# jmabuin/metacache-mpi

Hardware: AMD Instinct MI355X
Metric: query reads/sec (whole node) (higher is better)
Workload: dtype u32; 1 GPU; BASELINE configs[1]: 500 synthetic genomes (50 species x 10 strains, 2.0% divergence, 1.96 Gbp) in HBM, 1048576 x 150 bp single-end reads per step per GPU, k=16 s=16 w=128/113; reads_total=1632632832, db_keys=94389458, db_locations=277440620, db_hbm_bytes=34394191464, db_scaling=fixed, emulate_ranks=2, max_cand=2, P_x_M=4, distinct_batches=321, db_targets=500, parallelism=1 GPU, db_build_parts=1, remove_overpopulated_features=False

## Files before the change

### metacache-mpi_amd/csrc/mcq_device.hpp

```cpp
#pragma once
#include <cstddef>
#include <hip/hip_runtime.h>
#include <stdint.h>

typedef uint32_t u32;
typedef uint64_t u64;

#define MCQ_EMPTY 0xFFFFFFFFu
#ifndef MCQ_BLOCK_LONG_FIRST
#define MCQ_BLOCK_LONG_FIRST 16384u
#endif
#define MCQ_Q_UNPROBED 0x80000000u
#define MCQ_MAX_FOLD 64
#define MCQ_BIGLIST_MAX 1024u

namespace mcq {

struct DbDev {
    const uint4* slots;
    u32 slot_mask;
    u32 bsh;
    const void* locs;
    u32 wb;
    u32 compact;
// ... 51 lines not shown
        }
        t = lo; tb = o;
    }
    __device__ __forceinline__ u32 tbeg(u32 k) const { u32 t, tb; locate(k, t, tb); return tb; }
    __device__ __forceinline__ u32 tgt(u32 k) const { u32 t, tb; locate(k, t, tb); return t; }
};
template <class KeyT, bool GW> struct LocOf { typedef LocShift<KeyT> type; };
template <> struct LocOf<u32, true> { typedef LocGW type; };
template <class KeyT, bool GW>
__device__ __forceinline__ typename LocOf<KeyT, GW>::type loc_format(const DbDev& db, const GwDev& g) {
    if constexpr (GW) { LocGW f; f.off = g.off; f.blk = reinterpret_cast<const uint2*>(g.blk); f.shift = g.shift; return f; }
    else { LocShift<KeyT> f; f.wb = db.wb; return f; }
}
template <class KeyT>
__device__ __forceinline__ KeyT range_low(KeyT k, KeyT tb, u32 numWindows) {
    return (k - tb >= (KeyT)numWindows) ? k - (KeyT)(numWindows - 1) : tb;
}

struct BatchDev {
    const char* bases;
    const u64* seq_off;
    u64 n_seq;
    u64 nq;
    u32 paired;
    u32 ranges;
    u32 packed;
    u32 amb_off;
    u32 last_word;
    u32 amb_last;
};
__device__ __forceinline__ void seq_bounds(const u64* seq_off, u32 ranges, u64 a, u64& beg, u64& end) {
    if (ranges) { beg = seq_off[2 * a]; end = seq_off[2 * a + 1]; }
    else { beg = seq_off[a]; end = seq_off[a + 1]; }
}

struct OptDev {
    u32 max_cand;
    u32 P;
    u32 seg;
    u32 big;
    u32 quirk_seq_drop;
    u32 hooks;
    u64 insert_size_max;
    u32 n_fold;
    u32 n_levels;
    unsigned char level_end[8];
    unsigned char fold_snd[MCQ_MAX_FOLD];
    unsigned char fold_rcv[MCQ_MAX_FOLD];
    u64 tc_limit;
    u32 lin;
    u32 keep;
};
enum : u32 {
    MCQ_HOOK_BLOCK_ONLY   = 1u,
    MCQ_HOOK_RAW_SORT     = 2u,
    MCQ_HOOK_NO_WAVE16    = 4u,
    MCQ_HOOK_ROUTE        = MCQ_HOOK_BLOCK_ONLY | MCQ_HOOK_RAW_SORT | MCQ_HOOK_NO_WAVE16,
    MCQ_HOOK_ONLY_LAUNCH  = 8u,
    MCQ_HOOK_NO_TWO_CLASS = 16u,
    MCQ_HOOK_STOP_SHIFT   = 8u,
};
__device__ __host__ __forceinline__ bool two_class_lists(const OptDev& opt) {
    return (opt.lin ? opt.P <= 8u : opt.P * opt.max_cand <= 16u) && !(opt.hooks & MCQ_HOOK_NO_TWO_CLASS);
}

struct OutDev {
// ... 163 lines not shown
    static constexpr u32 W = MCQ_GEOM_DEFAULT_WINLEN, S = MCQ_GEOM_DEFAULT_STRIDE;
    __device__ __forceinline__ explicit GeomDefault(const DbDev&) {}
    __device__ __forceinline__ static constexpr u32 k() { return MCQ_GEOM_DEFAULT_K; }
    __device__ __forceinline__ static constexpr u32 s() { return MCQ_GEOM_DEFAULT_S; }
    __device__ __forceinline__ static constexpr u32 winlen() { return W; }
    __device__ __forceinline__ static constexpr u32 winstride() { return S; }
    __device__ __forceinline__ static constexpr u32 tgt_winstride() { return S; }
    __device__ __forceinline__ static u32 num_windows(u32 n) {
        if (n <= W) return 1;
        const u32 nfull = (n - W) / S + 1;
        return nfull + ((nfull * S < n) ? 1u : 0u);
    }
    __device__ __forceinline__ static void window_of(u32 n, u32 j, u32& beg, u32& len) {
        if (n <= W) { beg = 0; len = n; return; }
        const u32 nfull = (n - W) / S + 1;
        beg = j * S;
        len = (j < nfull) ? W : (n - beg);
    }
    __device__ __forceinline__ static u32 range_width(u64 qlen, u64 insert_size_max) {
        const u64 m = qlen > insert_size_max ? qlen : insert_size_max;
        if (m < (1ull << 31)) return 2 + (u32)m / S;
        return (u32)(2 + m / S);
    }
};
inline bool geom_is_default(const DbDev& d) {
    return d.k == MCQ_GEOM_DEFAULT_K && d.s == MCQ_GEOM_DEFAULT_S && d.winlen == MCQ_GEOM_DEFAULT_WINLEN &&
           d.winstride == MCQ_GEOM_DEFAULT_STRIDE && d.tgt_winstride == MCQ_GEOM_DEFAULT_STRIDE;
}
struct BatchRt {
    const BatchDev& b;
    __device__ __forceinline__ explicit BatchRt(const BatchDev& x) : b(x) {}
    __device__ __forceinline__ bool paired() const { return b.paired != 0; }
    __device__ __forceinline__ bool packed() const { return b.packed != 0; }
};
template <bool PAIRED, bool PACKED>
struct BatchForm {
    __device__ __forceinline__ explicit BatchForm(const BatchDev&) {}
    __device__ __forceinline__ static constexpr bool paired() { return PAIRED; }
    __device__ __forceinline__ static constexpr bool packed() { return PACKED; }
};

__device__ __forceinline__ u32 lane_rank(u64 mask) {
    return __builtin_amdgcn_mbcnt_hi((u32)(mask >> 32), __builtin_amdgcn_mbcnt_lo((u32)mask, 0u));
}

__device__ __forceinline__ void wave_sync() {
    __builtin_amdgcn_fence(__ATOMIC_RELEASE, "wavefront");
    __builtin_amdgcn_wave_barrier();
    __builtin_amdgcn_fence(__ATOMIC_ACQUIRE, "wavefront");
}

template <int CTRL>
__device__ __forceinline__ u32 dpp_mov(u32 v) {
    return (u32)__builtin_amdgcn_mov_dpp((int)v, CTRL, 0xF, 0xF, false);
}

__device__ __forceinline__ u32 wave_min_u32(u32 v) {
    u32 t;
    t = dpp_mov<0xB1>(v);  v = t < v ? t : v;
    t = dpp_mov<0x4E>(v);  v = t < v ? t : v;
    t = dpp_mov<0x141>(v); v = t < v ? t : v;
    t = dpp_mov<0x140>(v); v = t < v ? t : v;
    u32 a = __builtin_amdgcn_readlane(v, 0), b = __builtin_amdgcn_readlane(v, 16);
    u32 c = __builtin_amdgcn_readlane(v, 32), d = __builtin_amdgcn_readlane(v, 48);
    a = a < b ? a : b; c = c < d ? c : d;
    return a < c ? a : c;
}

__device__ __forceinline__ u32 bcast(u32 v, u32 src_lane) {
    return __builtin_amdgcn_readlane(v, src_lane);
}

// ... 295 lines not shown
    if (F(b).packed()) wave_words_of_packed(b, at, lane, w, am);
    else { u32 c0, c1; window_chars(b.bases + at, n, lane, c0, c1); wave_words_of_chars(c0, c1, lane, w, am); }
    return wave_sketch_words(w, am, n, k, s, lane, tmp, dst);
}

#ifndef MCQ_SKETCH_EXPECT_FUSED
#define MCQ_SKETCH_EXPECT_FUSED 25
#endif
struct __attribute__((packed)) PackedU32 { u32 v; };
__device__ __forceinline__ void encode_chars4(u32 c, u32& code8, u32& amb4) {
    const u32 z = (c & 0xDFDFDFDFu) ^ 0x41414141u;
    const u32 r = (z >> 1) & 0x03030303u;
    const u32 t = r & ~(r << 1) & 0x02020202u;
    const u32 bad = (z & 0xF9F9F9F9u) ^ ((t >> 1) | (t << 3));
    const u32 f = ((((bad & 0x7F7F7F7Fu) + 0x7F7F7F7Fu) | bad) >> 7) & 0x01010101u;
    const u32 x = r ^ ((r >> 1) & 0x01010101u);
    const u32 px = (x << 2) | (x >> 8);
    code8 = ((px << 4) | (px >> 16)) & 0xFFu;
    const u32 pf = (f << 1) | (f >> 8);
    amb4 = ((pf << 2) | (pf >> 16)) & 0xFu;
}
template <bool WIDE>
__device__ __forceinline__ u32 sketch_sorted_prefix(const u32* tmp, u32 cnt, u32 cap, u32 lane, u32* dst) {
    u32 v = lane < cnt ? tmp[lane] : MCQ_EMPTY;
    v = WIDE ? wave_sort64_1(v) : wave_sort_blocks32_1(v);
    asm("s_nop 1" : "+v"(v));
    const u32 prev = (u32)__builtin_amdgcn_update_dpp(0, (int)v, 0x138, 0xF, 0xF, false);
    const bool keep = (v != MCQ_EMPTY) && (lane == 0 || v != prev);
    const u64 km = __ballot(keep);
    const u32 rank = lane_rank(km);
    if (keep && rank < cap) dst[rank] = v;
    return (u32)__builtin_popcountll(km);
}
template <u32 E = MCQ_SKETCH_EXPECT_FUSED, bool REMAT = false>
__device__ __forceinline__ u32 wave_sketch_two_windows(const char* __restrict__ seq, u32 n, u32 lane, u32* tmp, u32* dst, u32& path) {
    if constexpr (REMAT) asm volatile("" : "+v"(lane));
    constexpr u32 K = MCQ_GEOM_DEFAULT_K, S = MCQ_GEOM_DEFAULT_S, W = MCQ_GEOM_DEFAULT_WINLEN, ST = MCQ_GEOM_DEFAULT_STRIDE;
    static_assert(K == 16 && S == 16 && W == 128 && ST == W - K + 1, "the two windows' k-mers partition; a k-mer is one 32-bit word");
    const u32 p4 = 4 * lane;
    const u32 la = p4 < n - 4 ? p4 : n - 4;
    u32 c = reinterpret_cast<const PackedU32*>(seq + la)->v >> (8 * ((p4 - la) & 3u));
    if (p4 >= n) c = 0;
    u32 code8, amb4;
    encode_chars4(c, code8, amb4);
    u32 w = code8 << (24 - 8 * (lane & 3));
    w |= xor_lane<1>(w, lane); w |= xor_lane<2>(w, lane);
    u32 am = amb4 << (28 - 4 * (lane & 7));
    am |= xor_lane<1>(am, lane); am |= xor_lane<2>(am, lane); am |= xor_lane<4>(am, lane);
    const u32 sh = (lane & 15) * 2, ash = lane & 31;
    const u32 wsrc = (lane & 0x30u), asrc = (lane & 0x20u);
    u32 h[3];
#pragma unroll
    for (int i = 0; i < 3; ++i) {
        const u32 pos = lane + 64 * i;
        const u32 w0 = (u32)__builtin_amdgcn_ds_bpermute((int)(wsrc + 64 * i), (int)w);
        const u32 w1 = (u32)__builtin_amdgcn_ds_bpermute((int)(wsrc + 64 * i + 16), (int)w);
        const u32 kmer = (u32)((((u64)w0 << 32) | w1) >> (32 - sh));
        const u32 m0 = (u32)__builtin_amdgcn_ds_bpermute((int)(asrc + 64 * i), (int)am);
        const u32 m1 = (u32)__builtin_amdgcn_ds_bpermute((int)(asrc + 64 * i + 32), (int)am);
        const u32 amb32 = (u32)((((u64)m0 << 32) | m1) >> (32 - ash));
        const bool ok = (i == 0 || pos + K <= n) && (amb32 >> (32 - K)) == 0;
        h[i] = ok ? tmh(canonical(kmer, K)) : MCQ_EMPTY;
    }
    const bool b1 = lane >= ST - 64;
    const u32 ha0 = h[0], ha1 = b1 ? MCQ_EMPTY : h[1], hb = b1 ? h[1] : h[2];
    const u32 cA = (u32)__builtin_popcountll(__ballot(ha0 != MCQ_EMPTY)) + (u32)__builtin_popcountll(__ballot(ha1 != MCQ_EMPTY));
    const bool all_in = cA <= 32;
    const u32 thr = all_in ? MCQ_EMPTY : (u32)fminf(__builtin_amdgcn_rcpf((float)cA) * (4294967296.0f * E), 4294967040.0f);
    const bool s0 = ha0 < thr, s1 = ha1 < thr, sb = hb != MCQ_EMPTY;
    const u64 m0 = __ballot(s0), m1 = __ballot(s1), mb = __ballot(sb);
    const u32 n0 = (u32)__builtin_popcountll(m0), cntA = n0 + (u32)__builtin_popcountll(m1), cntB = (u32)__builtin_popcountll(mb);
    const u32 capB = n - W;
    const u32 slB = capB < S ? capB : S;
    path = 0;
    if (cntA <= 32) {
        if (s0) tmp[lane_rank(m0)] = ha0;
        if (s1) tmp[n0 + lane_rank(m1)] = ha1;
        if (sb) tmp[32 + lane_rank(mb)] = hb;
        wave_sync();
        const bool hi = lane >= 32;
        u32 v = lane < (hi ? 32 + cntB : cntA) ? tmp[lane] : MCQ_EMPTY;
        v = wave_sort_blocks32_1(v);
        asm("s_nop 1" : "+v"(v));
        const u32 prev = (u32)__builtin_amdgcn_update_dpp(0, (int)v, 0x138, 0xF, 0xF, false);
        const bool keep = (v != MCQ_EMPTY) && ((lane & 31) == 0 || v != prev);
        const u64 km = __ballot(keep);
        const u32 DA = (u32)__builtin_popcount((u32)km), DB = (u32)__builtin_popcount((u32)(km >> 32));
        if (all_in || DA >= S) {
            const u32 mA = DA < S ? DA : S, mB = DB < slB ? DB : slB;
            const u32 rank = lane_rank(km) - (hi ? DA : 0u);
            if (keep && rank < (hi ? mB : mA)) dst[rank + (hi ? mA : 0u)] = v;
            wave_sync();
            return mA + mB;
        }
        wave_sync();
    }
    u32 mA = 0;
    bool exact = cntA > 64 || cntA <= 32;
    if (!exact) {
        path = 1;
        if (s0) tmp[lane_rank(m0)] = ha0;
        if (s1) tmp[n0 + lane_rank(m1)] = ha1;
        wave_sync();
        const u32 DA = sketch_sorted_prefix<true>(tmp, cntA, S, lane, dst);
        if (DA < S) exact = true; else mA = S;
        wave_sync();
    }
    if (exact) {
        path = 2;
        u32 a0 = ha0, a1 = ha1;
        for (mA = 0; mA < S; ++mA) {
            const u32 lo = a0 < a1 ? a0 : a1;
            const u32 mn = wave_min_u32(lo);
            if (mn == MCQ_EMPTY) break;
            if (lane == 0) dst[mA] = mn;
            if (a0 == mn) a0 = MCQ_EMPTY;
            if (a1 == mn) a1 = MCQ_EMPTY;
        }
// ... 1151 lines not shown
```

### metacache-mpi_amd/csrc/mcq_engine.hip

```cpp
#include "mcq_internal.hpp"

static thread_local std::string g_err;
extern "C" const char* mcq_last_error(void) { return g_err.c_str(); }
int mcq::set_error(int code, const char* msg) { g_err = msg; return code; }
extern "C" const char* mcq_version(void) { return "mcq 0.1 (gfx950)"; }

template <class Kernel>
static u32 resident_blocks(Kernel kernel, int block_size, int device) {
    int per_cu = 0;
    hipDeviceProp_t prop;
    if (hipOccupancyMaxActiveBlocksPerMultiprocessor(&per_cu, kernel, block_size, 0) != hipSuccess || per_cu < 1) per_cu = 4;
    if (hipGetDeviceProperties(&prop, device) != hipSuccess || prop.multiProcessorCount < 1) prop.multiProcessorCount = 256;
    if (const char* e = getenv("MCQ_WAVE_BLOCKS_PER_CU")) per_cu = std::max(1, atoi(e));
    return std::min<u32>((u32)per_cu * (u32)prop.multiProcessorCount, 8192u);
}
static u32 grid_for(u32 cap, u64 want) { return (u32)std::min<u64>(want ? want : 1, cap ? cap : 1); }

#define MCQ_LCAP_WAVE16 1024
__device__ __forceinline__ u32 pow2ceil(u32 x) { return x <= 1 ? 1u : 1u << (32 - __builtin_clz(x - 1)); }

template <class KeyT> __device__ __forceinline__ KeyT key_pad() { return ~(KeyT)0; }
template <class KeyT, class LF> __device__ __forceinline__ u64 key_expand(KeyT k, const LF& lf) {
    u32 t; KeyT tb;
    lf.locate(k, t, tb);
// ... 119 lines not shown
        if (D <= 64) return topk_lin_write<u32, 9, LF::lookup>(db, opt, out, sk, H, D, lf, q, lane, t1);
        return topk_lin_write<u32, 9>(db, opt, out, sk, H, D, lf, q, lane);
    }
    if (D > 64) {
        u32 nheads = 0;
        for (u32 base = 0; base < D; base += 64) {
            const u32 j = base + lane;
            const u32 hv = (j < D) ? H[j] : 0;
            const u64 hm = __ballot(hv != 0);
            if (hv != 0) H[nheads + lane_rank(hm)] = hv;
            nheads += (u32)__builtin_popcountll(hm);
        }
        wave_sync();
        return topk_all_lds<9, 4>(db, opt, out, sk, H, nheads, numWindows, lf, q, lane, H + 256);
    }
    return topk_fold_write_lds<9, LF::lookup>(db, opt, out, sk, H, D, numWindows, lf, q, lane, H + 256, t1);
}
#ifdef MCQ_PHASE_CLOCK
__shared__ u64 g_wph[4][12];
#define WCLK(i) do { asm volatile("s_waitcnt vmcnt(0) lgkmcnt(0)" ::: "memory"); if ((threadIdx.x & 63) == 0) { const u64 t_ = __builtin_amdgcn_s_memtime(); \
    u64* p_ = g_wph[threadIdx.x >> 6]; p_[i] += t_ - p_[11]; p_[11] = t_; } } while (0)
#else
#define WCLK(i) do { } while (0)
#endif
__device__ __forceinline__ u32 dedup_slot(u32 key) { return (key * 0x9E3779B1u) >> 23; }
__device__ __forceinline__ u32* dedup_sk(u32* hits) { return hits + 256; }
__device__ __forceinline__ u32* dedup_wp(u32* hits) { return hits; }
__device__ __forceinline__ u32 dedup_count(const u32* tabkey, const u32* tabcnt, u32 k) {
    u32 slot = dedup_slot(k);
    while (tabkey[slot] != k) slot = (slot + 1) & 511u;
    return (tabcnt[slot >> 1] >> (16 * (slot & 1))) & 0xFFFFu;
}

template <int E>
__device__ __forceinline__ u32 dedup_insert(const u32 (&r)[E], u32* buf, u32* hits, u32 T, u32 lane) {
    u32* tabkey = buf; u32* tabcnt = hits; u32* list = hits + 256;
    reinterpret_cast<uint4*>(tabkey)[lane] = make_uint4(MCQ_EMPTY, MCQ_EMPTY, MCQ_EMPTY, MCQ_EMPTY);
    reinterpret_cast<uint4*>(tabkey)[64 + lane] = make_uint4(MCQ_EMPTY, MCQ_EMPTY, MCQ_EMPTY, MCQ_EMPTY);
    u32 zero;
    asm volatile("v_mov_b32 %0, 0" : "=v"(zero));
    reinterpret_cast<uint4*>(tabcnt)[lane] = make_uint4(zero, zero, zero, zero);
    wave_sync();
    u32 D = 0;
#pragma unroll
    for (int e = 0; e < E; ++e) {
        if (e > 0 && (u32)(e * 64) >= T) break;
        const u32 key = r[e];
        bool created = false;
        if ((u32)(e * 64) + lane < T) {
            u32 slot = dedup_slot(key);
            while (true) {
                const u32 old = atomicCAS(&tabkey[slot], MCQ_EMPTY, key);
                created = old == MCQ_EMPTY;
                if (created || old == key) { atomicAdd(&tabcnt[slot >> 1], 1u << (16 * (slot & 1))); break; }
                slot = (slot + 1) & 511u;
            }
        }
        const u64 cm = __ballot(created);
        const u32 rank = D + lane_rank(cm);
        if (created && rank < MCQ_DEDUP_MAX_D) list[rank] = key;
        D += (u32)__builtin_popcountll(cm);
        if (D > MCQ_DEDUP_MAX_D) break;
    }
    wave_sync();
    return D;
}
template <class LF>
__device__ __forceinline__ u32 dedup_finish(u32 D, u32* buf, u32* hits, u32 lane, const LF& lf, u32& k1, u32& incl1, u32& t1, u32& tb1) {
    u32* tabkey = buf; u32* tabcnt = hits; u32* list = hits + 256; u32* SK = dedup_sk(hits); u32* WP = dedup_wp(hits);
    k1 = MCQ_EMPTY; incl1 = 0; t1 = 0; tb1 = 0;
    if (D > MCQ_DEDUP_MAX_D) return ~0u;
// ... 3 lines not shown
        if constexpr (LF::lookup) lf.locate(lane < D ? k : list[0], t1, tb1);
        const u32 c = lane < D ? dedup_count(tabkey, tabcnt, k) : 0u;
        const u32 incl = wave_incl_scan_dpp(c);
        wave_sync();
        SK[lane] = k; WP[lane] = incl;
        k1 = k; incl1 = incl;
    } else if (D <= 128) {
        u32 k[2];
        k[0] = list[lane]; k[1] = (64 + lane < D) ? list[64 + lane] : MCQ_EMPTY;
        wave_regsort<u32, 2>(k, lane);
        const u32 c0 = dedup_count(tabkey, tabcnt, k[0]);
        const u32 c1 = (64 + lane < D) ? dedup_count(tabkey, tabcnt, k[1]) : 0u;
        const u32 i0 = wave_incl_scan_dpp(c0);
        const u32 i1 = wave_incl_scan_dpp(c1) + bcast(i0, 63);
        wave_sync();
        SK[lane] = k[0]; SK[64 + lane] = k[1]; WP[lane] = i0; WP[64 + lane] = i1;
    } else {
        u32 k[4], c[4];
#pragma unroll
        for (int e = 0; e < 4; ++e) k[e] = ((u32)(64 * e) + lane < D) ? list[64 * e + lane] : MCQ_EMPTY;
        wave_regsort<u32, 4>(k, lane);
#pragma unroll
        for (int e = 0; e < 4; ++e) c[e] = ((u32)(64 * e) + lane < D) ? dedup_count(tabkey, tabcnt, k[e]) : 0u;
        u32 carry = 0;
#pragma unroll
        for (int e = 0; e < 4; ++e) { c[e] = wave_incl_scan_dpp(c[e]) + carry; carry = bcast(c[e], 63); }
        wave_sync();
#pragma unroll
        for (int e = 0; e < 4; ++e) { SK[64 * e + lane] = k[e]; WP[64 * e + lane] = c[e]; }
    }
    wave_sync();
    return D;
}
template <int E>
__device__ __forceinline__ u32 gather_dedup_insert(const DbDev& db, u32* buf, u32* hits, u32 T, u32 pos, u32 len, u64 off, u32 lane, int stop) {
    u32 r[E];
    gather_regs<u32, E>(db, r, T, pos, len, off, lane, hits);
    if (stop == 3) {
        u32 x = 0;
#pragma unroll
        for (int e = 0; e < E; ++e) x ^= r[e];
        buf[lane] = x;
        return ~1u;
    }
    return dedup_insert<E>(r, buf, hits, T, lane);
}
template <int E>
__device__ __forceinline__ u32 gather2_dedup_insert(const DbDev& db, u32* buf, u32* hits, u32 T, u32 pos0, u32 len0, u64 off0,
                                                    u32 pos1, u32 len1, u64 off1, bool two, u32 lane) {
    u32 r[E];
    gather_regs2<E>(db, r, T, pos0, len0, off0, pos1, len1, off1, two, lane, hits);
    return dedup_insert<E>(r, buf, hits, T, lane);
}
template <int E>
__device__ __forceinline__ u32 load_dedup_insert(const u32* __restrict__ src, u32* buf, u32* hits, u32 T, u32 lane) {
    u32 r[E];
#pragma unroll
    for (int e = 0; e < E; ++e) { const u32 t = e * 64 + lane; r[e] = t < T ? src[t] : MCQ_EMPTY; }
    return dedup_insert<E>(r, buf, hits, T, lane);
}

template <int E, class LF>
__device__ __forceinline__ bool heavy_sweep(u32 nH, u32 numWindows, const LF& lf, u32 lane, u32* buf, u32* hits, u32& D, u32*& SK, u32*& H, bool& nine) {
    constexpr int JB = 10;
    D = 0; SK = dedup_sk(hits); H = buf; nine = true;
    if (nH) {
        u32 rh[E];
#pragma unroll
        for (int e = 0; e < E; ++e) { const u32 t = e * 64 + lane; rh[e] = t < nH ? hits[t] : MCQ_EMPTY; }
        wave_sync();
        u32 k1 = MCQ_EMPTY, incl1 = 0, t1 = 0, tb1 = 0;
        const u32 Dd = dedup_insert<E>(rh, buf, hits, nH, lane);
        WCLK(4);
        if (E > 16 && Dd > MCQ_DEDUP_MAX_D) return false;
        if (E <= 4 || Dd <= MCQ_DEDUP_MAX_D) {
            D = dedup_finish(Dd, buf, hits, lane, lf, k1, incl1, t1, tb1);
            if (D <= 64 && numWindows <= 8) sweep_targets_regs(k1, incl1, tb1, H, D, numWindows, lf, lane);
            else sweep_targets_weighted(SK, dedup_wp(hits), H, D, numWindows, lf, lane);
// ... 82 lines not shown
    nL = T - nH;
    wave_sync();
    WCLK(3);
    if (nP > 64) return ~0u;
    const u32 safe = bcast(r[0], 0);
    const u32 lkey = lane < nP ? buf[lane] : MCQ_EMPTY;
    const bool omitted = nL > nP;
    u32 D, *SK, *H; bool nine, ok;
    if (nH <= 64)       ok = heavy_sweep<1>(nH, numWindows, lf, lane, buf, hits, D, SK, H, nine);
    else if (nH <= 128) ok = heavy_sweep<2>(nH, numWindows, lf, lane, buf, hits, D, SK, H, nine);
    else if (nH <= 256) ok = heavy_sweep<4>(nH, numWindows, lf, lane, buf, hits, D, SK, H, nine);
    else if (nH <= 512) ok = heavy_sweep<8>(nH, numWindows, lf, lane, buf, hits, D, SK, H, nine);
    else if (E > 8 && nH <= 1024) { if constexpr (E > 8) ok = heavy_sweep<16>(nH, numWindows, lf, lane, buf, hits, D, SK, H, nine); }
    else if (E > 16 && nH <= 2048) { if constexpr (E > 16) ok = heavy_sweep<32>(nH, numWindows, lf, lane, buf, hits, D, SK, H, nine); }
    else return ~1u;
    if (!ok) return ~1u;
    return heavy_lists(db, opt, out, D, SK, H, nine, lkey, omitted, theta, safe, numWindows, lf, q, lane);
}

struct ReadGeom {
    u64 o0, o1;
    u32 n1, n2;
    u32 nw1, nw2;
    u64 qlen;
    bool ovf;
    bool wide;
};
template <class G = GeomRt, class F = BatchRt>
__device__ __forceinline__ ReadGeom read_geom(const DbDev& db, const BatchDev& b, u64 q, bool block_only) {
    ReadGeom g;
    const G geo(db); const F form(b);
    const u64 a = form.paired() ? 2 * q : q;
    u64 e0, e1;
    seq_bounds(b.seq_off, b.ranges, a, g.o0, e0);
    if (form.paired()) seq_bounds(b.seq_off, b.ranges, a + 1, g.o1, e1); else { g.o1 = e0; e1 = e0; }
    const u64 l1 = e0 - g.o0, l2 = e1 - g.o1;
    g.qlen = l1 + l2;
    g.ovf = block_only || ((l1 | l2) >> 20) != 0;
    g.n1 = (u32)l1; g.n2 = (u32)l2; g.nw1 = 0; g.nw2 = 0; g.wide = false;
    if (!g.ovf) {
        g.nw1 = geo.num_windows(g.n1);
        g.nw2 = form.paired() ? geo.num_windows(g.n2) : 0;
        g.ovf = (g.nw1 + g.nw2) * geo.s() > 64;
        g.wide = g.ovf && (g.nw1 + g.nw2) * geo.s() <= 128;
    }
    return g;
}
template <class G = GeomRt>
__device__ __forceinline__ void window_span(const DbDev& db, const ReadGeom& g, u32 w, u64& at, u32& wl) {
    const bool m2 = w >= g.nw1;
    u32 beg;
    G(db).window_of(m2 ? g.n2 : g.n1, m2 ? w - g.nw1 : w, beg, wl);
    at = (m2 ? g.o1 : g.o0) + beg;
}
template <int JB, int CAP, class LF, class DB>
__device__ __forceinline__ u32 topk_heads(const DB& db, const OptDev& opt, const OutDev& out, const u32* buf, u32* hits,
                                          u32 T, u32 numWindows, const LF& lf, u64 q, u32 lane) {
    u32 nheads = 0;
    for (u32 base = 0; base < T; base += 64) {
        const u32 j = base + lane;
        const u32 hv = (j < T) ? hits[j] : 0;
        const u64 hm = __ballot(hv != 0);
        if (hv != 0) hits[nheads + lane_rank(hm)] = hv;
        nheads += (u32)__builtin_popcountll(hm);
    }
    wave_sync();
    if (opt.lin != 0) return topk_lin_write<u32, JB>(db, opt, out, buf, hits, nheads, lf, q, lane);
    constexpr int NC = CAP / 128;
// ... 37 lines not shown
template <class LF>
__device__ __forceinline__ void tap_distinct(const DebugDev& dbg, const u32* SK, const u32* WP, u32 D, const LF& lf, u64 q, u32 lane) {
    for (u32 j = lane; j < D; j += 64) {
        const u64 v = key_expand<u32>(SK[j], lf);
        for (u32 c = j ? WP[j - 1] : 0u; c < WP[j]; ++c) dbg.matches[dbg.match_off[q] + c] = v;
    }
}

template <class KeyT, int LCAP, bool TAP = false, bool SH = false, bool GW = false, int BSH = -1, int NL = 1, bool LEAN = false, bool EXCL = false,
          bool PAIRED = false, bool PACKED = false>
__global__ __launch_bounds__(256, sizeof(KeyT) == 4 ? (NL > 1 ? 5 : MCQ_WAVE_OCC) : 5) void k_query_wave(DbDev db, BatchDev b, OptDev opt, OutDev out,
                                                    CountersDev* ctr, u32* ovf_list, DebugDev dbg, ShardDev sh, GwDev gwd, ExclDev exd) {
    static_assert(LCAP == 512, "wave path: 8 keys per lane at most, entry index packed into 9 bits");
    static_assert(!GW || sizeof(KeyT) == 4, "the global-window form is a 32-bit word");
    static_assert(!LEAN || (sizeof(KeyT) == 4 && !TAP && !SH && NL == 1), "the lean form: 32-bit words, plain launches");
    static_assert(!EXCL || (!TAP && !SH && NL == 1 && !LEAN), "clade exclusion: plain launches of the full form, lists in a wave's lanes");
    static_assert(LEAN || (!PAIRED && !PACKED), "only the lean form knows the batch's form at compile time");
    using G = std::conditional_t<LEAN, GeomDefault, GeomRt>;
    using F = std::conditional_t<LEAN, BatchForm<PAIRED, PACKED>, BatchRt>;
    const G geo(db);
    constexpr u32 kKeepT = LEAN ? 256u : (u32)LCAP;
    if (!(opt.hooks & MCQ_HOOK_ONLY_LAUNCH) && ((ctr->direct_mode & MCQ_MODE_LEAN) != 0) != LEAN) return;
    using LF = typename LocOf<KeyT, GW>::type;
    const LF lf = loc_format<KeyT, GW>(db, gwd);
    const u32 hooks = LEAN ? 0u : opt.hooks;
    __shared__ KeyT s_buf[4][LCAP];
    __shared__ u32 s_hits[4][LCAP];
    const u32 lane = threadIdx.x & 63;
    const u32 wave = __builtin_amdgcn_readfirstlane(threadIdx.x >> 6);
    KeyT* buf = s_buf[wave];
    u32* hits = s_hits[wave];
    u32* sk_tmp = hits;
    u32* feat = hits + 64;
    const u64 nwaves = (u64)gridDim.x * 4;
    unsigned long long st_feat = 0, st_hit = 0, st_loc = 0, st_cand = 0;
    u32 st_geom = 0, st_long = 0;
#ifdef MCQ_PROFILE_HOOKS
    const int stop = (int)(hooks >> MCQ_HOOK_STOP_SHIFT);
#else
    constexpr int stop = 0;
#endif
    __shared__ u32 s_ovf[4][5];
    if (lane == 0) ovf_init(s_ovf[wave]);
    __shared__ u32 s_lean[4];
    if (lane == 0) s_lean[wave] = 0;
    __shared__ u32 s_tfail[4];
    if (!LEAN && lane == 0) s_tfail[wave] = MCQ_DEDUP_MAX_T + 1;
    wave_sync();

    if constexpr (sizeof(KeyT) == 4 && !TAP && NL == 1 && !LEAN) {
        if ((ctr->direct_mode & (SH ? MCQ_MODE_DIRECT_QUEUED : MCQ_MODE_DIRECT_GEOM)) && !(hooks & MCQ_HOOK_ROUTE) && stop == 0) {
            for (u64 q0 = ((u64)blockIdx.x * 4 + wave) * 64; q0 < b.nq; q0 += nwaves * 64) {
                const u64 q = q0 + lane;
                const bool valid = q < b.nq;
                bool front = false, lng = false;
                if (valid) { const ReadGeom g = read_geom(db, b, q, false); front = g.ovf && !g.wide; lng = MCQ_BLOCK_LONG_FIRST && g.qlen >= MCQ_BLOCK_LONG_FIRST; }
#pragma unroll
                for (int back = 0; back < 2; ++back) {
                    const u64 m = __ballot(valid && (back ? !front : front));
                    const u32 cnt = (u32)__builtin_popcountll(m);
                    if (!cnt) continue;
                    const u32 padded = (cnt + MCQ_OVF_CHUNK - 1) / MCQ_OVF_CHUNK * MCQ_OVF_CHUNK;
                    u32 base = 0;
                    if (lane == 0) base = atomicAdd(back ? &ctr->ovf_mid_count : &ctr->ovf_count, padded);
                    base = bcast(base, 0);
                    if (valid && (back ? !front : front)) ovf_list[ovf_slot(b.nq, back, base + lane_rank(m))] = (u32)q | (back ? MCQ_Q_UNPROBED : 0u);
                    if (lane < padded - cnt) ovf_list[ovf_slot(b.nq, back, base + cnt + lane)] = MCQ_EMPTY;
                }
                const u32 nv = (u32)__builtin_popcountll(__ballot(valid)), nf = (u32)__builtin_popcountll(__ballot(valid && front));
                const u32 nl = (u32)__builtin_popcountll(__ballot(lng));
                if (lane == 0) { atomicAdd(&ctr->n_ovf, nv); if (nf) atomicAdd(&ctr->n_geom, (unsigned long long)nf); if (nl) atomicAdd(&ctr->n_long, (unsigned long long)nl); }
            }
            return;
        }
    }
    for (u64 q = (u64)blockIdx.x * 4 + wave; q < b.nq; q += nwaves) {
        const ReadGeom g = read_geom<G, F>(db, b, q, (hooks & MCQ_HOOK_BLOCK_ONLY) != 0);
        bool ovf = g.ovf;
        u32 myf = MCQ_EMPTY, nfeat = 0, T = 0, len = 0, pos = 0;
        u64 off = 0;
        if (!ovf) {
            if constexpr (SH) {
                nfeat = (g.nw1 + g.nw2) * db.s;
                if (lane < nfeat) shard_fetch(sh, sh.win_off[b.paired ? 2 * q : q] * db.s + lane, off, len);
            } else {
            if constexpr (LEAN && !PAIRED && !PACKED) {
                if (g.n1 - 129u <= 31u) { u32 path; nfeat = wave_sketch_two_windows<MCQ_SKETCH_EXPECT_FUSED, GW>(b.bases + g.o0, g.n1, lane, sk_tmp, feat, path); }
                else for (u32 w = 0; w < g.nw1; ++w) {
                    u64 at; u32 wl;
                    window_span<G>(db, g, w, at, wl);
                    nfeat += wave_sketch_b<F>(b, at, wl, geo.k(), geo.s(), lane, sk_tmp, feat + nfeat);
                }
            } else
            for (u32 w = 0; w < g.nw1 + g.nw2; ++w) {
                u64 at; u32 wl;
                window_span<G>(db, g, w, at, wl);
                nfeat += wave_sketch_b<F>(b, at, wl, geo.k(), geo.s(), lane, sk_tmp, feat + nfeat);
            }
            if (lane < nfeat) myf = feat[lane];
            if (stop == 1) { if (myf == 12345u) out.ncand[q] = nfeat; continue; }
            probe<BSH>(db, myf, off, len);
            if (stop == 2) { if (len == 0x7FFFFFFFu) out.ncand[q] = (u32)off; continue; }
            }
            u32 incl = wave_incl_scan_dpp(len);
            pos = incl - len;
            T = bcast(incl, 63);
            if (T > kKeepT) ovf = true;
        }
        if (ovf) {
            if (LEAN && !g.ovf && T <= (u32)LCAP && lane == 0) s_lean[wave] += 1;
            if (g.ovf && !g.wide) ++st_geom;
            if (MCQ_BLOCK_LONG_FIRST && g.qlen >= MCQ_BLOCK_LONG_FIRST) ++st_long;
            if (sizeof(KeyT) == 4 && !g.ovf && T <= (u32)MCQ_LCAP_WAVE16 && !(hooks & MCQ_HOOK_NO_WAVE16)) {
                ovf_hand_over(s_ovf[wave], ctr, ovf_list, b.nq, (u32)q, off, len, lane);
                if constexpr (!SH) st_feat += nfeat;
                st_hit += (u32)__builtin_popcountll(__ballot(len > 0));
            } else {
                if (lane == 0) ovf_push(s_ovf[wave], (sizeof(KeyT) == 4 && g.wide && !(hooks & MCQ_HOOK_NO_WAVE16)) ? 1 : 0, ctr, ovf_list, b.nq, (u32)q);
                if constexpr (sizeof(KeyT) == 4 && !SH) {
                    if (!g.ovf && opt.tc_limit != 0) {
                        wave_sync();
                        const u32 slot = s_ovf[wave][0] - 1;
                        ctr->probe_front[(u64)slot * 64 + lane] = lane < nfeat ? ((off << 16) | len) : 0xFFFFull;
                    }
                }
            }
            continue;
        }
        if constexpr (!SH) st_feat += nfeat;
        st_hit += (u32)__builtin_popcountll(__ballot(len > 0)); st_loc += T;
        if constexpr (TAP) { if (dbg.mode == 1 && lane == 0) dbg.match_cnt[q] = T; }
        if (T == 0) { if (lane == 0) out.ncand[q] = 0; continue; }

        wave_sync();
        const u32 numWindows = geo.range_width(g.qlen, opt.insert_size_max);
        const auto& hdb = heads_db<EXCL>(db, exd, q);
        if constexpr (sizeof(KeyT) == 4) {
            if (LEAN || (T <= MCQ_DEDUP_MAX_T && !(hooks & MCQ_HOOK_RAW_SORT))) {
                u32 D = 0, k1 = MCQ_EMPTY, incl1 = 0, t1 = 0, tb1 = 0;
                bool skipped = false;
                if (T <= 64)       D = gather_dedup_insert<1>(db, buf, hits, T, pos, len, off, lane, stop);
                else if (T <= 128) D = gather_dedup_insert<2>(db, buf, hits, T, pos, len, off, lane, stop);
                else if (T <= 192) D = gather_dedup_insert<3>(db, buf, hits, T, pos, len, off, lane, stop);
                else if (LEAN || T <= 256) D = gather_dedup_insert<4>(db, buf, hits, T, pos, len, off, lane, stop);
                else if constexpr (!LEAN) {
                    if (lane == 0) s_lean[wave] += 1;
                    const u32 t_fail = s_tfail[wave];
                    skipped = T >= t_fail;
                    if (skipped) {
                        if (lane == 0) s_tfail[wave] = t_fail + 2;
                        D = MCQ_DEDUP_MAX_D + 1;
                    }
                    else if (T <= 384) D = gather_dedup_insert<6>(db, buf, hits, T, pos, len, off, lane, stop);
                    else               D = gather_dedup_insert<8>(db, buf, hits, T, pos, len, off, lane, stop);
                }
                if (D != ~1u) D = dedup_finish(D, buf, hits, lane, lf, k1, incl1, t1, tb1);
                if (stop == 3 || stop == 4) { if (buf[lane] == 0x1234u && D == 77u) out.ncand[q] = 1; wave_sync(); continue; }
                if (LEAN || D != ~0u) {
                    if constexpr (TAP) { if (dbg.mode == 2) tap_distinct(dbg, dedup_sk(hits), dedup_wp(hits), D, lf, q, lane); }
                    if (D <= 64 && numWindows <= 8) sweep_targets_regs(k1, incl1, tb1, reinterpret_cast<u32*>(buf), D, numWindows, lf, lane);
                    else sweep_targets_weighted(dedup_sk(hits), dedup_wp(hits), reinterpret_cast<u32*>(buf), D, numWindows, lf, lane);
                    if (stop == 5) { if (buf[lane] == 0x12345u) out.ncand[q] = 1; wave_sync(); continue; }
                    if constexpr (NL > 1) {
                        const u32 nc = topk_many_lists<NL>(db, opt, out, dedup_sk(hits), reinterpret_cast<u32*>(buf), D, numWindows, lf, q, lane, reinterpret_cast<u32*>(buf) + 256);
                        if (nc == ~0u) {
                            if (lane == 0) ovf_push(s_ovf[wave], 0, ctr, ovf_list, b.nq, (u32)q);
                            if constexpr (!SH) st_feat -= nfeat;
                            st_hit -= (u32)__builtin_popcountll(__ballot(len > 0)); st_loc -= T;
                        } else st_cand += nc;
                    } else
                    st_cand += topk_dedup(hdb, opt, out, dedup_sk(hits), reinterpret_cast<u32*>(buf), D, numWindows, lf, q, lane, t1);
                    wave_sync();
                    continue;
                }
                wave_sync();
                if (lane == 0 && !skipped) s_tfail[wave] = T;
            }
        }
        if constexpr (!LEAN) {
            if (T <= 64)       gather_sort_store<KeyT, 1>(db, buf, hits, T, pos, len, off, lane, stop);
            else if (T <= 128) gather_sort_store<KeyT, 2>(db, buf, hits, T, pos, len, off, lane, stop);
            else if (T <= 256) gather_sort_store<KeyT, 4>(db, buf, hits, T, pos, len, off, lane, stop);
            else               gather_sort_store<KeyT, 8>(db, buf, hits, T, pos, len, off, lane, stop);
            wave_sync();
            if (stop == 3 || stop == 4) { if (buf[lane] == (KeyT)0x1234) out.ncand[q] = 1; continue; }
            if constexpr (TAP) { if (dbg.mode == 2) tap_sorted<KeyT>(dbg, buf, T, lf, q, lane); }
            sweep_targets_wave<KeyT>(buf, hits, T, numWindows, lf, lane);
            if (stop == 5) { if (hits[lane] == 0x12345u) out.ncand[q] = 1; continue; }
            if constexpr (NL > 1) {
                const u32 nc = topk_many_lists<NL>(db, opt, out, reinterpret_cast<const u32*>(buf), hits, T, numWindows, lf, q, lane, hits + (LCAP - 128));
                if (nc == ~0u) {
                    if (lane == 0) ovf_push(s_ovf[wave], 0, ctr, ovf_list, b.nq, (u32)q);
                    if constexpr (!SH) st_feat -= nfeat;
                    st_hit -= (u32)__builtin_popcountll(__ballot(len > 0)); st_loc -= T;
                } else st_cand += nc;
            } else
            if constexpr (sizeof(KeyT) == 4) st_cand += topk_heads<9, LCAP>(hdb, opt, out, reinterpret_cast<const u32*>(buf), hits, T, numWindows, lf, q, lane);
            else st_cand += topk_heads64<KeyT>(hdb, opt, out, buf, hits, T, numWindows, lf, q, lane);
            wave_sync();
        }
    }
    if (lane == 0 && s_lean[wave]) atomicAdd(LEAN ? &ctr->n_lean : &ctr->n_lean_would, s_lean[wave]);
    if (lane == 0) ovf_flush(s_ovf[wave], ctr, ovf_list, b.nq);
    if (lane == 0 && st_geom) atomicAdd(&ctr->n_geom, (unsigned long long)st_geom);
    if (lane == 0 && st_long) atomicAdd(&ctr->n_long, (unsigned long long)st_long);
    if (lane == 0 && (st_feat | st_loc | st_hit)) {
        if (st_feat) atomicAdd(&ctr->n_features, st_feat);
        atomicAdd(&ctr->n_hit_features, st_hit);
        atomicAdd(&ctr->n_locations, st_loc);
        atomicAdd(&ctr->n_cands, st_cand);
    }
}

#ifndef MCQ_WAVE16_OCC
#define MCQ_WAVE16_OCC 4
#endif
template <bool TAP = false, bool SH = false, bool GW = false, int BSH = -1, bool EXCL = false>
__global__ __launch_bounds__(256, MCQ_WAVE16_OCC) void k_query_wave16(DbDev db, BatchDev b, OptDev opt, OutDev out,
                                                                      CountersDev* ctr, u32* ovf_list, DebugDev dbg, ShardDev sh, GwDev gwd, ExclDev exd) {
    constexpr int LCAP = MCQ_LCAP_WAVE16, JB = 10;
    const typename LocOf<u32, GW>::type lf = loc_format<u32, GW>(db, gwd);
    __shared__ u32 s_buf[4][LCAP];
    __shared__ u32 s_hits[4][LCAP];
    const u32 lane = threadIdx.x & 63;
    const u32 wave = __builtin_amdgcn_readfirstlane(threadIdx.x >> 6);
    u32* buf = s_buf[wave];
    u32* hits = s_hits[wave];
    u32* sk_tmp = hits;
    u32* feat = hits + 64;
    const u32 nwaves = gridDim.x * 4;
    const u32 n_mid = ctr->ovf_mid_count;
    unsigned long long st_feat = 0, st_hit = 0, st_loc = 0, st_cand = 0, st_two = 0, st_retry = 0, st_short = 0;
#ifdef MCQ_PHASE_CLOCK
    if (lane < 12) g_wph[wave][lane] = lane == 11 ? (u64)__builtin_amdgcn_s_memtime() : 0;
    wave_sync();
#endif
    u32 fq_next = 0, fq_left = 0;
    float word_space;
    if constexpr (GW) word_space = (float)gwd.off[db.n_targets];
    else word_space = (db.wb < 32 && ((u64)db.n_targets << db.wb) < 0xFFFFFFFFull) ? (float)((u64)db.n_targets << db.wb) : 4294967040.0f;
    for (u32 it = blockIdx.x * 4 + wave; it < n_mid; it += nwaves) {
        WCLK(7);
        const u32 qe = ovf_list[ovf_slot(b.nq, 1, ovf_visit(it, n_mid))];
// ... 905 lines not shown
}

int mcq::launch_query(const mcq_db* db, mcq_ws* ws, const BatchDev& b, const OptDev& od_in, const OutDev& o,
                      hipStream_t st, LeanReq lean_req, const DebugDev& dbg, const ShardDev* shp, const DbDev* dbd, const ExclDev* exp) {
    if (!shp) HIPCHK(hipMemsetAsync(ws->ctr.get(), 0, MCQ_CTR_ZEROED, st));
    if (b.nq == 0) return MCQ_OK;
    const ShardDev sh = shp ? *shp : ShardDev{};
    const DbDev& D = dbd ? *dbd : db->d;
    const u64 want = (b.nq + 3) / 4;
    const u32 grid = grid_for(ws->cap_wave, want);
    LaunchTimer tm(ws, st);
    int rc = tm.begin(); if (rc) return rc;
    const bool tap = dbg.mode != 0;
    const ExclDev ex = exp ? *exp : ExclDev{};
    LaunchPlan p; rc = plan_launch(db, od_in, tap, shp != nullptr, exp != nullptr, lean_req, p); if (rc) return rc;
    const OptDev& od = p.rest;
    using Yes = std::true_type; using No = std::false_type;
    auto by_role = [&](auto f) {
        if (shp) f(No{}, Yes{}, IntC<-1>{}, No{});
        else if (tap) f(Yes{}, No{}, IntC<-1>{}, No{});
        else if (exp) f(No{}, No{}, IntC<-1>{}, Yes{});
        else with_layout(db, [&](auto BSH) { f(No{}, No{}, BSH, No{}); });
    };
    rc = with_loc_form(db, [&](auto L) -> int {
        using Key = typename decltype(L)::Key;
        constexpr bool GW = decltype(L)::gw;
        auto first = [&](auto TAP, auto SH, auto BSH, auto NL, auto LEAN, auto EX, u32 g, auto PAIRED, auto PACKED) {
            hipLaunchKernelGGL((k_query_wave<Key, kLcapWave, TAP, SH, GW, BSH, NL, LEAN, EX, PAIRED, PACKED>), dim3(g), dim3(256), 0, st, D, b, p.first, o, ws->ctr.get(), ws->ovf_list.get(), dbg, sh, db->g, ex);
        };
        if (p.full) by_role([&](auto TAP, auto SH, auto BSH, auto EX) { first(TAP, SH, BSH, IntC<1>{}, No{}, EX, grid, No{}, No{}); });
        if constexpr (sizeof(Key) == 4) {
            if (p.many) with_layout(db, [&](auto BSH) { first(No{}, No{}, BSH, IntC<4>{}, No{}, No{}, grid_for(ws->cap_wave_many, want), No{}, No{}); });
            if (p.lean) with_layout(db, [&](auto BSH) {
                auto lean = [&](auto PAIRED, auto PACKED) { first(No{}, No{}, BSH, IntC<1>{}, Yes{}, No{}, grid, PAIRED, PACKED); };
                if (b.paired) { if (b.packed) lean(Yes{}, Yes{}); else lean(Yes{}, No{}); }
                else { if (b.packed) lean(No{}, Yes{}); else lean(No{}, No{}); }
            });
        }
        rc = tm.mark(); if (rc) return rc;
        if constexpr (sizeof(Key) == 4) {
            by_role([&](auto TAP, auto SH, auto BSH, auto EX) {
                hipLaunchKernelGGL((k_query_wave16<TAP, SH, GW, BSH, EX>), dim3(grid_for(ws->cap_wave16, want)), dim3(256), 0, st, D, b, od, o, ws->ctr.get(),
                                   ws->ovf_list.get(), dbg, sh, db->g, ex);
            });
            if (p.with_tc) by_role([&](auto TAP, auto SH, auto BSH, auto EX) {
                if constexpr (!TAP && !EX) hipLaunchKernelGGL((k_query_wave32<SH, GW, BSH>), dim3(grid_for(ws->cap_wave32, want)), dim3(256), 0, st, D, b, od, o,
                                                       ws->ctr.get(), ws->ovf_list.get(), sh, db->g);
            });
        }
        rc = tm.mark(); if (rc) return rc;
        constexpr int lcap = sizeof(Key) == 4 ? MCQ_BLOCK_LCAP : kLcapBlock, nt = sizeof(Key) == 4 ? MCQ_BLOCK_NT : 1024;
        auto block = [&](auto TC, auto BIG) {
            auto launch = [&](auto SH, auto EX) {
                if constexpr (!(EX && TC)) hipLaunchKernelGGL((k_query_block<Key, lcap, nt, BIG, SH, GW, TC, EX>), dim3(ws->n_block_wgs), dim3(nt), 0, st, D, b, od, o, ws->ctr.get(),
                                   (const u32*)ws->ovf_list.get(), ws->sc, dbg, sh, db->g, ex);
            };
            if (shp) launch(Yes{}, No{}); else if (exp) launch(No{}, Yes{}); else launch(No{}, No{});
        };
        if (od.lin) block(No{}, IntC<2>{}); else if (od.big) block(No{}, IntC<1>{}); else block(No{}, IntC<0>{});
        if constexpr (sizeof(Key) == 4) if (p.with_tc) { if (od.lin) block(Yes{}, IntC<2>{}); else block(Yes{}, IntC<0>{}); }
        return MCQ_OK;
    });
    if (rc) return rc;
    rc = tm.end(); if (rc) return rc;
    if (p.next_mode) hipLaunchKernelGGL(k_next_mode, dim3(1), dim3(1), 0, st, ws->ctr.get(), b.nq, (p.full && p.lean) ? 1u : 0u);
    else HIPCHK(hipMemsetAsync(&ws->ctr.get()->direct_mode, 0, 4, st));
    HIPCHK(hipGetLastError());
// ... 361 lines not shown
```

Before: 643.1 million reads/s.

## Narrow lean-kernel indices to 32-bit and load read bounds through scalar constant path

In the lean wave kernel, the read index, stride and per-wave counters become 32-bit, and the number of windows is precomputed from insert_size_max outside the loop. Read offsets are loaded through a constant (scalar) address space pointer for the templated batch form. Asm barriers rematerialise lane masks and the empty literal to cut register pressure. The lean grid is enlarged so the 32-bit index cannot overflow. Together these aim to lower VGPR/SGPR use and per-read scalar overhead, at the risk of miscompiling the uniform-load assumption or hitting 32-bit limits.

```diff
diff --git a/metacache-mpi_amd/csrc/mcq_device.hpp b/metacache-mpi_amd/csrc/mcq_device.hpp
--- a/metacache-mpi_amd/csrc/mcq_device.hpp
+++ b/metacache-mpi_amd/csrc/mcq_device.hpp
@@ -107,6 +107,11 @@
 __device__ __forceinline__ void seq_bounds(const u64* seq_off, u32 ranges, u64 a, u64& beg, u64& end) {
     if (ranges) { beg = seq_off[2 * a]; end = seq_off[2 * a + 1]; }
     else { beg = seq_off[a]; end = seq_off[a + 1]; }
+}
+__device__ __forceinline__ void seq_bounds_uniform(const u64* seq_off, u32 ranges, u64 a, u64& beg, u64& end) {
+    typedef const u64 __attribute__((address_space(4))) * ConstU64;
+    const ConstU64 p = (ConstU64)(uintptr_t)seq_off + (ranges ? 2 * a : a);
+    beg = p[0]; end = p[1];
 }
 
 struct OptDev {
@@ -336,12 +341,14 @@
     __device__ __forceinline__ explicit BatchRt(const BatchDev& x) : b(x) {}
     __device__ __forceinline__ bool paired() const { return b.paired != 0; }
     __device__ __forceinline__ bool packed() const { return b.packed != 0; }
+    __device__ __forceinline__ static void seq_bounds(const u64* seq_off, u32 ranges, u64 a, u64& beg, u64& end) { mcq::seq_bounds(seq_off, ranges, a, beg, end); }
 };
 template <bool PAIRED, bool PACKED>
 struct BatchForm {
     __device__ __forceinline__ explicit BatchForm(const BatchDev&) {}
     __device__ __forceinline__ static constexpr bool paired() { return PAIRED; }
     __device__ __forceinline__ static constexpr bool packed() { return PACKED; }
+    __device__ __forceinline__ static void seq_bounds(const u64* seq_off, u32 ranges, u64 a, u64& beg, u64& end) { seq_bounds_uniform(seq_off, ranges, a, beg, end); }
 };
 
 __device__ __forceinline__ u32 lane_rank(u64 mask) {
@@ -703,7 +710,7 @@
     if (keep && rank < cap) dst[rank] = v;
     return (u32)__builtin_popcountll(km);
 }
-template <u32 E = MCQ_SKETCH_EXPECT_FUSED, bool REMAT = false>
+template <u32 E = MCQ_SKETCH_EXPECT_FUSED, bool REMAT = false, bool REMAT_MASKS = false>
 __device__ __forceinline__ u32 wave_sketch_two_windows(const char* __restrict__ seq, u32 n, u32 lane, u32* tmp, u32* dst, u32& path) {
     if constexpr (REMAT) asm volatile("" : "+v"(lane));
     constexpr u32 K = MCQ_GEOM_DEFAULT_K, S = MCQ_GEOM_DEFAULT_S, W = MCQ_GEOM_DEFAULT_WINLEN, ST = MCQ_GEOM_DEFAULT_STRIDE;
@@ -733,7 +740,9 @@
         const bool ok = (i == 0 || pos + K <= n) && (amb32 >> (32 - K)) == 0;
         h[i] = ok ? tmh(canonical(kmer, K)) : MCQ_EMPTY;
     }
-    const bool b1 = lane >= ST - 64;
+    u32 ln = lane;
+    if constexpr (REMAT_MASKS) asm volatile("" : "+v"(ln));
+    const bool b1 = ln >= ST - 64;
     const u32 ha0 = h[0], ha1 = b1 ? MCQ_EMPTY : h[1], hb = b1 ? h[1] : h[2];
     const u32 cA = (u32)__builtin_popcountll(__ballot(ha0 != MCQ_EMPTY)) + (u32)__builtin_popcountll(__ballot(ha1 != MCQ_EMPTY));
     const bool all_in = cA <= 32;
@@ -749,12 +758,12 @@
         if (s1) tmp[n0 + lane_rank(m1)] = ha1;
         if (sb) tmp[32 + lane_rank(mb)] = hb;
         wave_sync();
-        const bool hi = lane >= 32;
+        const bool hi = ln >= 32;
         u32 v = lane < (hi ? 32 + cntB : cntA) ? tmp[lane] : MCQ_EMPTY;
         v = wave_sort_blocks32_1(v);
         asm("s_nop 1" : "+v"(v));
         const u32 prev = (u32)__builtin_amdgcn_update_dpp(0, (int)v, 0x138, 0xF, 0xF, false);
-        const bool keep = (v != MCQ_EMPTY) && ((lane & 31) == 0 || v != prev);
+        const bool keep = (v != MCQ_EMPTY) && ((ln & 31) == 0 || v != prev);
         const u64 km = __ballot(keep);
         const u32 DA = (u32)__builtin_popcount((u32)km), DB = (u32)__builtin_popcount((u32)(km >> 32));
         if (all_in || DA >= S) {
diff --git a/metacache-mpi_amd/csrc/mcq_engine.hip b/metacache-mpi_amd/csrc/mcq_engine.hip
--- a/metacache-mpi_amd/csrc/mcq_engine.hip
+++ b/metacache-mpi_amd/csrc/mcq_engine.hip
@@ -175,11 +175,13 @@
     return (tabcnt[slot >> 1] >> (16 * (slot & 1))) & 0xFFFFu;
 }
 
-template <int E>
+template <int E, bool LIT = false>
 __device__ __forceinline__ u32 dedup_insert(const u32 (&r)[E], u32* buf, u32* hits, u32 T, u32 lane) {
     u32* tabkey = buf; u32* tabcnt = hits; u32* list = hits + 256;
-    reinterpret_cast<uint4*>(tabkey)[lane] = make_uint4(MCQ_EMPTY, MCQ_EMPTY, MCQ_EMPTY, MCQ_EMPTY);
-    reinterpret_cast<uint4*>(tabkey)[64 + lane] = make_uint4(MCQ_EMPTY, MCQ_EMPTY, MCQ_EMPTY, MCQ_EMPTY);
+    u32 empty = MCQ_EMPTY;
+    if constexpr (LIT) asm volatile("v_mov_b32 %0, -1" : "=v"(empty));
+    reinterpret_cast<uint4*>(tabkey)[lane] = make_uint4(empty, empty, empty, empty);
+    reinterpret_cast<uint4*>(tabkey)[64 + lane] = make_uint4(empty, empty, empty, empty);
     u32 zero;
     asm volatile("v_mov_b32 %0, 0" : "=v"(zero));
     reinterpret_cast<uint4*>(tabcnt)[lane] = make_uint4(zero, zero, zero, zero);
@@ -249,7 +251,7 @@
     wave_sync();
     return D;
 }
-template <int E>
+template <int E, bool LIT = false>
 __device__ __forceinline__ u32 gather_dedup_insert(const DbDev& db, u32* buf, u32* hits, u32 T, u32 pos, u32 len, u64 off, u32 lane, int stop) {
     u32 r[E];
     gather_regs<u32, E>(db, r, T, pos, len, off, lane, hits);
@@ -260,7 +262,7 @@
         buf[lane] = x;
         return ~1u;
     }
-    return dedup_insert<E>(r, buf, hits, T, lane);
+    return dedup_insert<E, LIT>(r, buf, hits, T, lane);
 }
 template <int E>
 __device__ __forceinline__ u32 gather2_dedup_insert(const DbDev& db, u32* buf, u32* hits, u32 T, u32 pos0, u32 len0, u64 off0,
@@ -409,8 +411,8 @@
     const G geo(db); const F form(b);
     const u64 a = form.paired() ? 2 * q : q;
     u64 e0, e1;
-    seq_bounds(b.seq_off, b.ranges, a, g.o0, e0);
-    if (form.paired()) seq_bounds(b.seq_off, b.ranges, a + 1, g.o1, e1); else { g.o1 = e0; e1 = e0; }
+    F::seq_bounds(b.seq_off, b.ranges, a, g.o0, e0);
+    if (form.paired()) F::seq_bounds(b.seq_off, b.ranges, a + 1, g.o1, e1); else { g.o1 = e0; e1 = e0; }
     const u64 l1 = e0 - g.o0, l2 = e1 - g.o1;
     g.qlen = l1 + l2;
     g.ovf = block_only || ((l1 | l2) >> 20) != 0;
@@ -514,8 +516,10 @@
     u32* hits = s_hits[wave];
     u32* sk_tmp = hits;
     u32* feat = hits + 64;
-    const u64 nwaves = (u64)gridDim.x * 4;
-    unsigned long long st_feat = 0, st_hit = 0, st_loc = 0, st_cand = 0;
+    using QI = std::conditional_t<LEAN, u32, u64>;
+    using ST = std::conditional_t<LEAN, u32, unsigned long long>;
+    const QI nwaves = (QI)gridDim.x * 4;
+    ST st_feat = 0, st_hit = 0, st_loc = 0, st_cand = 0;
     u32 st_geom = 0, st_long = 0;
 #ifdef MCQ_PROFILE_HOOKS
     const int stop = (int)(hooks >> MCQ_HOOK_STOP_SHIFT);
@@ -556,7 +560,10 @@
             return;
         }
     }
-    for (u64 q = (u64)blockIdx.x * 4 + wave; q < b.nq; q += nwaves) {
+    const QI nq = (QI)b.nq;
+    const bool ism_huge = LEAN && opt.insert_size_max >= (1ull << 31);
+    const u32 nw_ism = LEAN ? geo.range_width(0, opt.insert_size_max) : 0u;
+    for (QI q = (QI)blockIdx.x * 4 + wave; q < nq; q += nwaves) {
         const ReadGeom g = read_geom<G, F>(db, b, q, (hooks & MCQ_HOOK_BLOCK_ONLY) != 0);
         bool ovf = g.ovf;
         u32 myf = MCQ_EMPTY, nfeat = 0, T = 0, len = 0, pos = 0;
@@ -567,7 +574,7 @@
                 if (lane < nfeat) shard_fetch(sh, sh.win_off[b.paired ? 2 * q : q] * db.s + lane, off, len);
             } else {
             if constexpr (LEAN && !PAIRED && !PACKED) {
-                if (g.n1 - 129u <= 31u) { u32 path; nfeat = wave_sketch_two_windows<MCQ_SKETCH_EXPECT_FUSED, GW>(b.bases + g.o0, g.n1, lane, sk_tmp, feat, path); }
+                if (g.n1 - 129u <= 31u) { u32 path; nfeat = wave_sketch_two_windows<MCQ_SKETCH_EXPECT_FUSED, GW, true>(b.bases + g.o0, g.n1, lane, sk_tmp, feat, path); }
                 else for (u32 w = 0; w < g.nw1; ++w) {
                     u64 at; u32 wl;
                     window_span<G>(db, g, w, at, wl);
@@ -615,16 +622,20 @@
         if (T == 0) { if (lane == 0) out.ncand[q] = 0; continue; }
 
         wave_sync();
-        const u32 numWindows = geo.range_width(g.qlen, opt.insert_size_max);
+        u32 numWindows;
+        if constexpr (LEAN) {
+            const u32 nw_q = 2 + (u32)g.qlen / G::S;
+            numWindows = (ism_huge || nw_ism > nw_q) ? nw_ism : nw_q;
+        } else numWindows = geo.range_width(g.qlen, opt.insert_size_max);
         const auto& hdb = heads_db<EXCL>(db, exd, q);
         if constexpr (sizeof(KeyT) == 4) {
             if (LEAN || (T <= MCQ_DEDUP_MAX_T && !(hooks & MCQ_HOOK_RAW_SORT))) {
                 u32 D = 0, k1 = MCQ_EMPTY, incl1 = 0, t1 = 0, tb1 = 0;
                 bool skipped = false;
-                if (T <= 64)       D = gather_dedup_insert<1>(db, buf, hits, T, pos, len, off, lane, stop);
-                else if (T <= 128) D = gather_dedup_insert<2>(db, buf, hits, T, pos, len, off, lane, stop);
-                else if (T <= 192) D = gather_dedup_insert<3>(db, buf, hits, T, pos, len, off, lane, stop);
-                else if (LEAN || T <= 256) D = gather_dedup_insert<4>(db, buf, hits, T, pos, len, off, lane, stop);
+                if (T <= 64)       D = gather_dedup_insert<1, LEAN>(db, buf, hits, T, pos, len, off, lane, stop);
+                else if (T <= 128) D = gather_dedup_insert<2, LEAN>(db, buf, hits, T, pos, len, off, lane, stop);
+                else if (T <= 192) D = gather_dedup_insert<3, LEAN>(db, buf, hits, T, pos, len, off, lane, stop);
+                else if (LEAN || T <= 256) D = gather_dedup_insert<4, LEAN>(db, buf, hits, T, pos, len, off, lane, stop);
                 else if constexpr (!LEAN) {
                     if (lane == 0) s_lean[wave] += 1;
                     const u32 t_fail = s_tfail[wave];
@@ -687,10 +698,10 @@
     if (lane == 0 && st_geom) atomicAdd(&ctr->n_geom, (unsigned long long)st_geom);
     if (lane == 0 && st_long) atomicAdd(&ctr->n_long, (unsigned long long)st_long);
     if (lane == 0 && (st_feat | st_loc | st_hit)) {
-        if (st_feat) atomicAdd(&ctr->n_features, st_feat);
-        atomicAdd(&ctr->n_hit_features, st_hit);
-        atomicAdd(&ctr->n_locations, st_loc);
-        atomicAdd(&ctr->n_cands, st_cand);
+        if (st_feat) atomicAdd(&ctr->n_features, (unsigned long long)st_feat);
+        atomicAdd(&ctr->n_hit_features, (unsigned long long)st_hit);
+        atomicAdd(&ctr->n_locations, (unsigned long long)st_loc);
+        atomicAdd(&ctr->n_cands, (unsigned long long)st_cand);
     }
 }
 
@@ -1662,7 +1673,8 @@
         if constexpr (sizeof(Key) == 4) {
             if (p.many) with_layout(db, [&](auto BSH) { first(No{}, No{}, BSH, IntC<4>{}, No{}, No{}, grid_for(ws->cap_wave_many, want), No{}, No{}); });
             if (p.lean) with_layout(db, [&](auto BSH) {
-                auto lean = [&](auto PAIRED, auto PACKED) { first(No{}, No{}, BSH, IntC<1>{}, Yes{}, No{}, grid, PAIRED, PACKED); };
+                const u32 lean_grid = std::max<u32>(grid, (u32)(want >> 22) + 1);
+                auto lean = [&](auto PAIRED, auto PACKED) { first(No{}, No{}, BSH, IntC<1>{}, Yes{}, No{}, lean_grid, PAIRED, PACKED); };
                 if (b.paired) { if (b.packed) lean(Yes{}, Yes{}); else lean(Yes{}, No{}); }
                 else { if (b.packed) lean(No{}, Yes{}); else lean(No{}, No{}); }
             });
```

After: 659.3 million reads/s, median of 6. 2.5% higher.
